# weecology/DeepTreeAttention

Hardware: AMD Instinct MI355X
Metric: patches/sec (train step) Hang2020 369-band 11x11 (higher is better)
Workload: dtype bf16; 1 GPU; Hang2020 spectral+spatial attention train step (fwd + weighted CE + bwd + Adam), bands=369 11x11 classes=200; per_gpu_batch=1024, global_batch=1024, parallelism=dp1, overlap_comm=False, ranks_seen=1

## Files before the change

deeptreeattention_amd/csrc/capi.hip:

```cpp
#include <math.h>
#include <stdlib.h>
#include <stdarg.h>
#include <stdio.h>
#include <string.h>

#include "../../include/dta_hip.h"
#include "kernels.h"
#include "xchg_dev.h"

using namespace dta;

extern "C" {
int dta_xchg_side_args(dta_xchg* x, const double* alpha_g, long long alpha_slot, dta::XchgArgs* out);
void dta_xchg_side_cancel(dta_xchg* x);
}

static thread_local char g_err[512] = "";
void dta_set_error(const char* fmt, ...) {
  va_list ap;
  va_start(ap, fmt);
  vsnprintf(g_err, sizeof(g_err), fmt, ap);
  va_end(ap);
}

// ... 309 lines not shown
  ca.B = p.B; ca.H = p.Hc[L]; ca.W = p.Wc[L]; ca.NC = p.NCin[L]; ca.N = Nconv; ca.Q = p.Qin[L]; ca.HW = p.HWc[L];
  return ca;
}
ConvArgs dgrad_conv_geom(const Plan& p, int L) {
  ConvArgs ca;
  memset(&ca, 0, sizeof(ca));
  ca.B = p.B; ca.H = p.Hc[L]; ca.W = p.Wc[L]; ca.NC = CH[L] / 16; ca.N = CH[L - 1]; ca.Q = p.Qin[L]; ca.HW = p.HWc[L];
  return ca;
}
inline int conv_tab_slot_fwd(int L) { return L; }
inline int conv_tab_slot_dgrad(int L) { return 2 + L; }
void use_conv_tabs(const Plan& p, void* ws, ConvArgs& ca, int G, int slot) {
  if (p.esz != 2) return;
  const int rows = conv_bf16_rows(ca, G);
  if (rows <= 0 || ca.HW > rows) return;
  ca.tabs = reinterpret_cast<const int*>(reinterpret_cast<char*>(ws) + p.rowtabs + (size_t)slot * CONV_TAB_BYTES);
  ca.tabs_rows = rows;
}
bool add_conv_tab_job(const Plan& p, void* ws, const ConvArgs& geom, int G, int slot, ConvTabGroup& tg) {
  ConvArgs ca = geom;
  use_conv_tabs(p, ws, ca, G, slot);
  if (!ca.tabs) return false;
  ConvTabJob& j = tg.job[tg.n++];
  j.HW = ca.HW; j.W = ca.W; j.Q = ca.Q; j.rows = ca.tabs_rows; j.ppw = ca.tabs_rows / ca.HW; j.order = switches().conv_order;
  j.dst = const_cast<int*>(ca.tabs);
  return true;
}

struct LossArgs { const long long* labels; const float* weight; float* loss; float* dlogits; float* scratch; };

struct FwdOpts {
  const void* x_tiles = nullptr;
  const float* gate = nullptr;
  const LossArgs* loss = nullptr;
  bool y0_ready = false;
};
struct BwdOpts {
  int phases = 3;
  const void* x_tiles = nullptr;
  float* dalpha32 = nullptr;
  const float* gate = nullptr;
  dta_xchg* xchg = nullptr;
  long long alpha_slot = -1;
};

bool tail_plan(const Plan& p, const dta_net_desc* d, float* const (*scores)[3]) {
  if (d->kind != DTA_NET_HANG2020 || !d->training || (d->heads_mask & 7) != 4 || (d->heads_mask & DTA_FORWARD_ONLY)) return false;
  if (switches().no_tail || switches().no_lean || !(switches().lean_mask & 1) || switches().bn_inkernel || (switches().fanin & 1)) return false;
  if (scores && (scores[0][2] || scores[1][2])) return false;
  if (p.H != 11 || p.W != 11 || p.F[0][2] != 128 || p.F[1][2] != 512) return false;
  return true;
}

template <typename T>
int forward_t(const Plan& p, const dta_net_desc* d, const dta_subnet_params* nets, const double* alpha,
              const float* const* xs, void* ws, float* const (*scores)[3], float* joint, hipStream_t st,
              const FwdOpts& o) {
  const void* x_tiles = o.x_tiles; const float* gate = o.gate; const LossArgs* loss = o.loss;
  if (o.y0_ready && (d->training || !(d->heads_mask & DTA_FORWARD_ONLY) || p.H != 11 || p.W != 11 || x_tiles)) {
    dta_set_error("a forward on a ready first-conv output needs eval mode, DTA_FORWARD_ONLY and 11x11 patches");
    return 1;
  }
  if (x_tiles && !(p.esz == 2 && p.x_compact && (p.shared_x || p.G == 1))) {
    dta_set_error("input tiles need the bf16 mode, 11x11-class patches and a single input tensor");
    return 1;
  }
  const int G = p.G, B = p.B;
  GemmGroup heads;
  bool tail = tail_plan(p, d, scores);
  if (tail) {
    StageArgs s3 = stage_args(p, d, nets, ws, 2);
    tail = tail_fwd_supported(s3, G, p.classes);
  }
  bool loss_done = false;
  PackWGroup packs;
  SpecPackGroup spacks;
  int pack_mode[3];
  for (int L = 0; L < 3; ++L) {
    const int C = CH[L];
    PackWArgs pw;
    memset(&pw, 0, sizeof(pw));
    const bool cat = L == 0 && p.shared_x;
    pw.G = cat ? 1 : G; pw.NC = p.NCin[L]; pw.N = cat ? 32 * G : C; pw.K = p.Cin[L];
    for (int g = 0; g < G; ++g) pw.src[g] = nets[g].conv_w[L];
    pw.mode = (cat && G == 2) ? 1 : 0; pw.nsplit = 32;
    pack_mode[L] = pw.mode;
    packs.job[packs.n] = pw; packs.dst[packs.n++] = at<char>(ws, p.wp[L]);
    if (L > 0 && d->training) {
      memset(&pw, 0, sizeof(pw));
      pw.G = G; pw.NC = C / 16; pw.N = CH[L - 1]; pw.K = C; pw.mode = 2;
      for (int g = 0; g < G; ++g) pw.src[g] = nets[g].conv_w[L];
      packs.job[packs.n] = pw; packs.dst[packs.n++] = at<char>(ws, p.wd[L]);
    }
    for (int g = 0; g < G; ++g)
      if (p.kinds[g] == KIND_SPECTRAL) {
        int j = spacks.n++;
        spacks.w1[j] = nets[g].att[L][0]; spacks.w2[j] = nets[g].att[L][2];
        spacks.packed[j] = at<float>(ws, p.attpk[g][L]); spacks.C[j] = C; spacks.K[j] = SPEC_K[L];
      }
  }
  const bool reuse = !d->training && (d->heads_mask & DTA_FORWARD_ONLY) && (d->heads_mask & DTA_REUSE_PACKED);
  if (reuse) { packs.n = 0; spacks.n = 0; }
  {
    PrepArgs pa = {};
    pa.nx = (x_tiles || o.y0_ready || fused_input(p)) ? 0 : (p.shared_x ? 1 : G); pa.x_tl_gs = p.x_tl_gs;
    for (int g = 0; g < pa.nx; ++g) pa.x[g] = xs[g];
    pa.x_tl = at<char>(ws, p.x_tl); pa.B = B; pa.C = p.bands; pa.H = p.H; pa.W = p.W;
    pa.x_compact = p.x_compact;
    pa.packs = packs; pa.spacks = spacks;
    if (sizeof(T) == 2 && !reuse) {
      const bool fan_fwd0 = d->training && (switches().fanin & 1);
      for (int L = o.y0_ready ? 1 : 0; L < 3; ++L) add_conv_tab_job(p, ws, fwd_conv_geom(p, d, L, fan_fwd0), (L == 0 && p.shared_x) ? 1 : G, conv_tab_slot_fwd(L), pa.tabs);
      if (d->training && !(d->heads_mask & DTA_FORWARD_ONLY))
        for (int L = 1; L < 3; ++L) add_conv_tab_job(p, ws, dgrad_conv_geom(p, L), G, conv_tab_slot_dgrad(L), pa.tabs);
    }
    if (tail) {
      for (int g = 0; g < 2; ++g) {
        if (!nets[g].fc_w[2] || !nets[g].fc_b[2]) { dta_set_error("Hang2020 forward: the last heads' parameters are missing"); return 1; }
        pa.trans.src[g] = nets[g].fc_w[2];
        pa.trans.dst[g] = at<float>(ws, p.fct) + (size_t)(g ? p.F[0][2] : 0) * p.fct_ld;
        pa.trans.rows[g] = p.classes; pa.trans.cols[g] = p.F[g][2]; pa.trans.ld[g] = p.fct_ld;
      }
      pa.trans.n = 2;
    }
    if (switches().fanin) { pa.zero = at<float>(ws, p.fan_cnt); pa.zero_n4 = (p.fan_cnt_bytes + (d->heads_mask ? p.scores_bytes : 0) + 15) / 16; }
    else { pa.zero = at<float>(ws, p.lead); pa.zero_n4 = (256 + (d->heads_mask ? p.scores_bytes : 0) + 15) / 16; }
    if (launch_forward_prep<T>(pa, st)) return 1;
  }
  for (int L = 0; L < 3; ++L) {
    const int C = CH[L];
    const bool cat = L == 0 && p.shared_x;
    const int Nconv = cat ? 32 * G : C;
    const int launchG = cat ? 1 : G;
    const bool fan_fwd = d->training && (switches().fanin & 1);
    ConvArgs ca = fwd_conv_geom(p, d, L, fan_fwd);
    use_conv_tabs(p, ws, ca, launchG, conv_tab_slot_fwd(L));
    ca.pixel_order = switches().conv_order;
    if (L == 0) {
      ca.x_tl = x_tiles ? x_tiles : at<char>(ws, p.x_tl); ca.x_gs = p.x_tl_gs / p.esz; ca.x_compact = p.x_compact;
      if (!x_tiles && fused_input(p)) {
        for (int g = 0; g < G; ++g) ca.x_nchw[g] = xs[p.shared_x ? 0 : g];
        ca.Cx = p.bands;
        ca.x_tl_out = (d->heads_mask & DTA_FORWARD_ONLY) ? nullptr : at<char>(ws, p.x_tl);
      }
    } else { ca.x_tl = at<char>(ws, p.a_tl[L - 1]); ca.x_gs = (size_t)B * p.NCin[L] * p.Rin[L] * 16; ca.x_compact = p.tl_compact; }
    ca.wp = at<char>(ws, p.wp[L]);
    for (int g = 0; g < G; ++g) ca.bias[g] = nets[g].conv_b[L];
    ca.bias_mode = pack_mode[L]; ca.bias_split = 32;
    ca.y = at<float>(ws, p.y[L]); ca.y_fmt = p.y_fmt;
    if (cat) { ca.y_gs = 0; ca.y_rs = Nconv; } else { ca.y_gs = (size_t)B * p.HWc[L] * C; ca.y_rs = C; }
    ca.stats = d->training ? at<float>(ws, p.stats[L]) : nullptr;
    if (fan_fwd) { ca.fan_count = at<unsigned>(ws, p.fan_ctr) + (size_t)L * MAXG * FAN_R; ca.fan_sums = at<double>(ws, p.fan_fwd[L]); }
    if (!(L == 0 && o.y0_ready)) {
      prof_begin(DTA_SITE_CONV_FWD + L, st);
      if (launch_conv3x3<T>(ca, launchG, st)) return 1;
      prof_end(DTA_SITE_CONV_FWD + L, st);
    }
    BnFinalizeArgs bf;
    memset(&bf, 0, sizeof(bf));
    bf.stats = at<float>(ws, p.stats[L]); bf.nwg = p.nwg[L]; bf.N = Nconv; bf.HW = p.HWc[L]; bf.MWG = p.MWG[L]; bf.B = B;
    for (int g = 0; g < G; ++g) {
      bf.gamma[g] = nets[g].bn_w[L]; bf.beta[g] = nets[g].bn_b[L];
      bf.rmean[g] = nets[g].bn_rm[L]; bf.rvar[g] = nets[g].bn_rv[L]; bf.nbt[g] = nets[g].bn_nbt[L];
    }
    bf.cat_mode = (cat && G == 2); bf.nsplit = 32;
    bf.coef = at<float>(ws, p.coef[L]); bf.training = d->training; bf.momentum = d->bn_momentum; bf.eps = d->bn_eps;
    bf.gate = gate;
    StageArgs sa = stage_args(p, d, nets, ws, L);
    if (fan_fwd) { bf.fsum = ca.fan_sums; sa.bn_inkernel = 1; sa.bnfin = bn_finalize_kargs(bf); }
    else if ((!d->training || switches().bn_inkernel) && p.nwg[L] <= BN_INKERNEL_MAX_NWG) { sa.bn_inkernel = 1; sa.bnfin = bn_finalize_kargs(bf); }
    else if ((switches().lead & 1) && !(L == 2 && tail) && stage_fwd_will_be_lean(sa, G)) {
      sa.bnfin = bn_finalize_kargs(bf);
      sa.lead = G * ((sa.bnfin.C + 7) / 8); sa.lead_flag = at<unsigned>(ws, p.lead) + L; sa.lead_need = (unsigned)sa.lead;
    }
    else if (launch_bn_finalize(bf, G, st)) return 1;
    if (d->heads_mask & DTA_FORWARD_ONLY) sa.attsave = nullptr;
    if (L == 2 && tail) {
      TailArgs ta;
      memset(&ta, 0, sizeof(ta));
      ta.st = sa;
      ta.wt = at<float>(ws, p.fct); ta.ldw = p.fct_ld;
      for (int g = 0; g < 2; ++g) { ta.bias[g] = nets[g].fc_b[2]; ta.scores[g] = at<float>(ws, p.scores[g][2]); }
      ta.alpha = alpha; ta.classes = p.classes;
      ta.ce.gscale = 1.f;
      if (loss) {
        if (!alpha) { dta_set_error("Hang2020 forward + loss needs alpha"); return 1; }
        ta.ce.labels = loss->labels; ta.ce.weight = loss->weight; ta.ce.loss = loss->loss; ta.ce.dlogits = loss->dlogits;
        ta.ce.rowtmp = loss->scratch; ta.ce.joint = joint;
        loss_done = true;
      } else if (!(d->heads_mask & DTA_SKIP_BLEND)) {
        if (!joint || !alpha) { dta_set_error("Hang2020 forward needs head 3, alpha and a joint output"); return 1; }
        ta.ce.joint = joint;
      }
      prof_begin(DTA_SITE_STAGE_FWD + L, st);
      if (launch_tail_fwd(ta, st)) return 1;
      prof_end(DTA_SITE_STAGE_FWD + L, st);
      continue;
    }
    prof_begin(DTA_SITE_STAGE_FWD + L, st);
    if (launch_stage_fwd<T>(sa, G, st)) return 1;
    prof_end(DTA_SITE_STAGE_FWD + L, st);
    if (d->heads_mask & (1 << L)) {
      for (int g = 0; g < G; ++g) {
        if (p.F[g][L] == 0 || nets[g].fc_w[L] == nullptr) continue;
        const int F = p.F[g][L];
        GemmArgs ga;
        memset(&ga, 0, sizeof(ga));
        ga.A = at<float>(ws, p.feat[L]) + (size_t)g * sa.feat_gs; ga.sa_m = F; ga.sa_k = 1;
        ga.Bm = nets[g].fc_w[L]; ga.sb_k = 1; ga.sb_n = F;
        float* out = at<float>(ws, p.scores[g][L]);
        ga.M = B; ga.N = p.cls[g]; ga.K = F; ga.ksplit = min(4, max(1, (F + 63) / 64)); ga.accumulate = 0;
        float* user = (scores && scores[g][L]) ? scores[g][L] : nullptr;
        if (d->kind == DTA_NET_VANILLA && joint) user = joint;
        if (user) {
          out = user;
          if (ga.ksplit > 1) hipMemsetAsync(user, 0, (size_t)B * p.cls[g] * 4, st);
        }
        ga.C = out; ga.sc_m = p.cls[g]; ga.sc_n = 1;
        ga.bias = nets[g].fc_b[L];
        if (!heads.add(ga)) { dta_set_error("too many head GEMMs"); return 1; }
      }
    }
  }
  prof_begin(DTA_SITE_GEMM, st);
  if (launch_gemm_group(heads, st)) return 1;
  prof_end(DTA_SITE_GEMM, st);
  if (tail) return (loss && !loss_done) ? 1 : 0;
  if (loss) {
    BlendCeArgs a;
    memset(&a, 0, sizeof(a));
    a.gscale = 1.f;
    if (d->kind == DTA_NET_HANG2020) {
      if (!alpha || !(d->heads_mask & 4)) { dta_set_error("Hang2020 forward + loss needs head 3 and alpha"); return 1; }
      a.spec = (scores && scores[0][2]) ? scores[0][2] : at<float>(ws, p.scores[0][2]);
      a.spat = (scores && scores[1][2]) ? scores[1][2] : at<float>(ws, p.scores[1][2]);
      a.alpha = alpha; a.joint = joint;
    } else {
      if (!joint) { dta_set_error("forward + loss: the scores of a single-branch network are passed in `joint`"); return 1; }
      a.spec = joint; a.joint = joint;
    }
    a.labels = loss->labels; a.weight = loss->weight; a.dlogits = loss->dlogits; a.loss = loss->loss; a.rowtmp = loss->scratch;
    a.B = B; a.classes = p.classes;
    return launch_blend_ce(a, st);
  }
  if (d->kind == DTA_NET_HANG2020 && !(d->heads_mask & DTA_SKIP_BLEND)) {
    if (!(d->heads_mask & 4) || !joint || !alpha) { dta_set_error("Hang2020 forward needs head 3, alpha and a joint output"); return 1; }
    BlendArgs ba;
    ba.spec = (scores && scores[0][2]) ? scores[0][2] : at<float>(ws, p.scores[0][2]);
    ba.spat = (scores && scores[1][2]) ? scores[1][2] : at<float>(ws, p.scores[1][2]);
    ba.alpha = alpha; ba.joint = joint; ba.B = B; ba.classes = p.classes;
    if (launch_blend(ba, st)) return 1;
  }
  return 0;
}

template <typename T>
int conv_wgrad_layer(const Plan& p, const dta_net_desc* d, const dta_subnet_grads* grads, void* ws, int L,
                     WgradReduceGroup& reduces, hipStream_t st, const BwdOpts& o, const double* dalpha,
                     WgradArgs* defer = nullptr, const WgradArgs* partner = nullptr) {
  const int G = p.G, B = p.B, C = CH[L];
  const bool cat = L == 0 && p.shared_x;
  const int Nconv = cat ? 32 * G : C;
  const int launchG = cat ? 1 : G;
  bool want_w = false;
// ... 1209 lines not shown
```

deeptreeattention_amd/csrc/conv.hip:

```cpp
#include <stdlib.h>

#include "kernels.h"

namespace dta {

template <typename T>
__device__ __forceinline__ void pack_input_block(const float* __restrict__ x, T* __restrict__ out, int B, int C, int H,
                                                 int W, int NC, int CG, int b, int ycg, unsigned char* smem,
                                                 bool compact = false) {
  const int HW = H * W, Q = (H + 2) * (W + 2);
  int* lut = (int*)smem;
  float* sbase = (float*)(lut + ((Q + 3) & ~3));
  const int chunk0 = ycg * CG;
  const int nch = min(CG, NC - chunk0);
  const int c0 = chunk0 * 16;
  const int creal = max(0, min(nch * 16, C - c0));
  const float* src = x + ((size_t)b * C + c0) * HW;
  for (int q = threadIdx.x; q < Q; q += 256) {
    int hh = q / (W + 2) - 1, ww = q % (W + 2) - 1;
    lut[q] = (hh >= 0 && hh < H && ww >= 0 && ww < W) ? hh * W + ww : -1;
  }
  const size_t e0 = ((size_t)b * C + c0) * HW;
  const int phase = (int)(e0 & 3);
  float* s = sbase + phase;
// ... 136 lines not shown
  conv_row_tables<ROWS, 256>(c, rowtab, plq, hist, flag, 0, j.ppw, 0);
  __syncthreads();
  for (int i = threadIdx.x; i < 2 * ROWS; i += 256) j.dst[i] = tab_s[i];
}
__device__ __forceinline__ void conv_tab_job(const ConvTabJob& j) {
  __shared__ int tab_s[2 * 576 + 256 + 4];
  if (j.rows == 256) conv_tab_rows<256>(j, tab_s);
  else if (j.rows == 512) conv_tab_rows<512>(j, tab_s);
  else if (j.rows == 576) conv_tab_rows<576>(j, tab_s);
}

template <typename T>
__global__ __launch_bounds__(256) void k_forward_prep(PrepArgs a) {
  extern __shared__ __attribute__((aligned(16))) unsigned char smem[];
  int y = blockIdx.y;
  if (a.tabs.n > 0) {
    if (y == 0) {
      if ((int)blockIdx.x < a.tabs.n) conv_tab_job(a.tabs.job[blockIdx.x]);
      return;
    }
    y -= 1;
  }
  if (y < a.ncg * a.nx) {
    const int gi = y / a.ncg;
    if ((int)blockIdx.x >= a.B) return;
    pack_input_block<T>(a.x[gi], (T*)((char*)a.x_tl + (size_t)gi * a.x_tl_gs), a.B, a.C, a.H, a.W, a.NC, a.CG, blockIdx.x,
                        y - gi * a.ncg, smem, a.x_compact != 0);
    return;
  }
  y -= a.ncg * a.nx;
  const size_t nthreads = (size_t)gridDim.x * blockDim.x, tid = blockIdx.x * (size_t)blockDim.x + threadIdx.x;
  if (y < a.packs.n) { pack_conv_w_job<T>(a.packs.job[y], (T*)a.packs.dst[y], tid, nthreads); return; }
  y -= a.packs.n;
  if (y < a.spacks.n) { pack_spectral_att_job(a.spacks, y, tid, nthreads); return; }
  y -= a.spacks.n;
  if (y < a.trans.n) { transpose_job(a.trans, y, tid, nthreads); return; }
  y -= a.trans.n;
  if (a.zero) {
    float4* z = (float4*)a.zero;
    for (size_t i = tid; i < a.zero_n4; i += nthreads) z[i] = make_float4(0.f, 0.f, 0.f, 0.f);
  }
}

template <typename T>
int launch_forward_prep(PrepArgs a, hipStream_t st) {
  size_t lds;
  if (pack_input_plan(a.C, a.H, a.W, &a.NC, &a.CG, &lds)) return 1;
  a.ncg = (a.NC + a.CG - 1) / a.CG;
  constexpr int PREP_MIN_BLOCKS = 1024;
  size_t most = a.zero ? a.zero_n4 : 0;
  for (int j = 0; j < a.packs.n; ++j) { const PackWArgs& w = a.packs.job[j]; const size_t e = (size_t)w.G * w.NC * 9 * w.N * 4; if (e > most) most = e; }
  for (int j = 0; j < a.spacks.n; ++j) { const size_t e = (size_t)a.spacks.C[j] * a.spacks.C[j]; if (e > most) most = e; }
  for (int j = 0; j < a.trans.n; ++j) { const size_t e = (size_t)a.trans.cols[j] * a.trans.ld[j]; if (e > most) most = e; }
  int gx = (int)((most + 1023) / 1024);
  gx = gx < 256 ? 256 : (gx > PREP_MIN_BLOCKS ? PREP_MIN_BLOCKS : gx);
  if (a.nx > 0 && gx < a.B) gx = a.B;
  dim3 grid(gx, a.ncg * a.nx + a.packs.n + a.spacks.n + a.trans.n + (a.tabs.n > 0 ? 1 : 0) + (a.zero ? 1 : 0));
  hipLaunchKernelGGL(k_forward_prep<T>, grid, dim3(256), lds, st, a);
  DTA_CHECK_LAUNCH("k_forward_prep");
  return 0;
}
template int launch_forward_prep<float>(PrepArgs, hipStream_t);
template int launch_forward_prep<bf16_t>(PrepArgs, hipStream_t);

template <typename T> struct Frag;
template <> struct Frag<float> {
  static constexpr int KS = 2;
  typedef float reg;
  __device__ static __forceinline__ reg load(const float* rowbase, int row, int ks, int lane) {
    return rowbase[tl_pos<float>(row, ks * 2 + (lane >> 5))];
  }
  __device__ static __forceinline__ f32x16 mfma(reg a, reg b, f32x16 c) {
    return __builtin_amdgcn_mfma_f32_32x32x2f32(a, b, c, 0, 0, 0);
  }
};
template <> struct Frag<bf16_t> {
  static constexpr int KS = 16;
  typedef bf16x8 reg;
  __device__ static __forceinline__ reg load(const bf16_t* rowbase, int row, int ks, int lane) {
    return *reinterpret_cast<const bf16x8*>(rowbase + tl_pos<bf16_t>(row, (lane >> 5) << 3));
  }
  __device__ static __forceinline__ f32x16 mfma(reg a, reg b, f32x16 c) {
    return __builtin_amdgcn_mfma_f32_32x32x16_bf16(a, b, c, 0, 0, 0);
  }
};

template <typename T, int MT, int NT>
__global__ __launch_bounds__(256, 2) void k_conv3x3(ConvArgs a) {
  extern __shared__ __attribute__((aligned(16))) unsigned char smem[];
  constexpr int MWG = 4 * MT * 32;
  constexpr int N = NT * 32;
  int* rowtab = (int*)smem;
  int* plq = rowtab + MWG;
  float* red = (float*)(plq + MWG);
  float* cmean = red + 4 * N;
  T* sx = (T*)(cmean + N);
  const int Q = a.Q, HW = a.HW, W2 = a.W + 2;
  T* sw = sx + (size_t)a.ppw * Q * 16;

  const int tid = threadIdx.x, lane = tid & 63, wave = tid >> 6;
  const int g = blockIdx.y;
  const int pg = blockIdx.x / a.spp, split = blockIdx.x - pg * a.spp;
  const int b0 = pg * a.ppw;
  const int npatch = min(a.ppw, a.B - b0);

  for (int lr = tid; lr < MWG; lr += 256) {
    int pl, pix;
    bool valid;
// ... 389 lines not shown
```

deeptreeattention_amd/csrc/conv_bf16.hip:

```cpp
#include <type_traits>
#include "kernels.h"
#include "xchg_dev.h"

namespace dta {

constexpr int RB = 48;
typedef __attribute__((address_space(3))) s16x4* lds_s16x4_t;

typedef __bf16 hw_bf16x2 __attribute__((ext_vector_type(2)));
__device__ __forceinline__ unsigned cvt_pk_bf16(float lo, float hi) {
  f32x2 v = {lo, hi};
  return __builtin_bit_cast(unsigned, __builtin_convertvector(v, hw_bf16x2));
}

__device__ __forceinline__ int fastdiv(int n, unsigned magic) { return (int)__umulhi((unsigned)n, magic); }
static inline unsigned fastdiv_magic(int d) { return d > 1 ? (unsigned)((0x100000000ull + (unsigned long long)d - 1) / (unsigned long long)d) : 0u; }
__device__ __forceinline__ int fastdiv1(int n, int d, unsigned magic) { return d > 1 ? fastdiv(n, magic) : n; }

__device__ __forceinline__ bf16x8 lds_b128(const unsigned char* base, int off) {
  return *reinterpret_cast<const bf16x8*>(base + off);
}
__device__ __forceinline__ bf16x8 lds_tr8(const unsigned char* base, int off) {
  s16x4 lo = __builtin_amdgcn_ds_read_tr16_b64_v4i16((lds_s16x4_t)(base + off));
  s16x4 hi = __builtin_amdgcn_ds_read_tr16_b64_v4i16((lds_s16x4_t)(base + off + 4 * RB));
// ... 30 lines not shown
#define XS_ACC { xsacc_[0] += xs_[1] - xs_[0]; xsacc_[1] += xs_[2] - xs_[1]; xsacc_[2] += xs_[3] - xs_[2]; }
#define XT(i) xt_[i] = clock64();
#define XT_ACC { _Pragma("unroll") for (int k_ = 0; k_ < 5; ++k_) xacc_[k_] += xt_[k_ + 1] - xt_[k_]; }
#else
#define XT(i)
#define XT_ACC
#define XS(i)
#define XS_ACC
#endif
#ifdef DTA_TICKS
__device__ long long g_cticks[16];
extern "C" int dta_debug_cticks(long long* out) { return (int)hipMemcpyFromSymbol(out, HIP_SYMBOL(g_cticks), sizeof(long long) * 16); }
#define CTICK(i) do { if (!XN && a.N == 64 && a.NC == 2 && a.stats && blockIdx.x == 100 && blockIdx.y == 0 && threadIdx.x == 0) g_cticks[i] = clock64(); } while (0)
#else
#define CTICK(i)
#endif
template <int MT, int NT, bool XN, int NWV = 8, int MINW = 1>
__global__ __launch_bounds__(NWV * 64, MINW) void k_conv3x3_bf16(ConvArgs a) {
  WGSTAMP(XN ? 0 : (a.stats ? (a.N == 64 ? 1 : 2) : -1));
  extern __shared__ __attribute__((aligned(16))) unsigned char smem[];
#ifdef DTA_TICKS
  const long long xentry_ = clock64();
#endif
  CTICK(0);
  constexpr int NW = NWV, NTHR = NW * 64;
  constexpr int MWG = NW * MT * 32;
  constexpr int N = NT * 32;
  constexpr bool TAP_PIPE = true;
  static_assert(!(XN && MT * NT >= 6), "six accumulator tiles + the fp32 staging sets spill (see launch_conv_bf16_t)");
  int* rowtab = (int*)smem;
  int* plq = rowtab + MWG;
  float* red = (float*)(plq + MWG);
  float* cmean = red + NW * N;
  unsigned char* sbuf = (unsigned char*)(cmean + N + NW * N);
  const int Q = a.Q, HW = a.HW, W2 = a.W + 2;
  const int xbytes = a.ppw * Q * RB, wbytes = 9 * N * RB, stage = xbytes + wbytes;
  const bool dbuf = a.dbuf != 0;

  const int tid = threadIdx.x, lane = tid & 63, wave = tid >> 6;
  const int g = blockIdx.y;
  const int pg = a.spp == 1 ? (int)blockIdx.x : (int)blockIdx.x / a.spp, split = blockIdx.x - pg * a.spp;
  const int b0 = pg * a.ppw;
  const int npatch = min(a.ppw, a.B - b0);

  int tab0_[2] = {-1, -1}, tab1_[2] = {0, 0};
  static_assert(MWG <= 2 * NTHR, "two table entries per thread at most");
  if (a.tabs && a.spp == 1 && npatch == a.ppw) {
#pragma unroll
    for (int k = 0; k < 2; ++k)
      if (tid + k * NTHR < MWG) { tab0_[k] = a.tabs[tid + k * NTHR]; tab1_[k] = a.tabs[MWG + tid + k * NTHR]; }
  }
  const int khalf16 = (lane >> 5) * 16;
  int abase[MT];
  const int bbase = (lane & 31) * RB + khalf16;
  const bool xc = a.x_compact != 0;
#define DTA_TABLES \
  { \
    if (a.tabs && a.spp == 1 && npatch == a.ppw) {    \
      _Pragma("unroll") for (int k_ = 0; k_ < 2; ++k_) {                                              \
        const int lr_ = tid + k_ * NTHR;                                                              \
        if (lr_ < MWG) { rowtab[lr_] = tab0_[k_] < 0 ? -1 : b0 * HW + tab0_[k_]; plq[lr_] = tab1_[k_]; } \
      }                                                                                               \
    } else conv_row_tables<MWG, NTHR>(a, rowtab, plq, reinterpret_cast<int*>(red), reinterpret_cast<int*>(cmean), b0, npatch, split); \
    if (xc || XN) {    \
      u32x4* z = reinterpret_cast<u32x4*>(sbuf); \
      const u32x4 zero = {0u, 0u, 0u, 0u}; \
      for (int i = tid; i < xbytes / 16; i += NTHR) { z[i] = zero; if (dbuf) z[i + stage / 16] = zero; } \
    } \
    __syncthreads(); \
_Pragma("unroll") \
    for (int mt = 0; mt < MT; ++mt) { \
      int v = plq[(wave * MT + mt) * 32 + (lane & 31)]; \
      abase[mt] = ((v >> 16) * Q + (v & 0xFFFF)) * RB + khalf16; \
    } \
  }
  if (XN) DTA_TABLES

  f32x16 acc[MT][NT];
#pragma unroll
  for (int mt = 0; mt < MT; ++mt)
#pragma unroll
    for (int nt = 0; nt < NT; ++nt)
#pragma unroll
      for (int r = 0; r < 16; ++r) acc[mt][nt][r] = 0.f;
  float bias[NT];
  if (!XN) {
#pragma unroll
    for (int nt = 0; nt < NT; ++nt) {
      const int n = nt * 32 + (lane & 31);
      float bv = 0.f;
      if (a.bias[0]) {
        if (a.bias_mode == 1) bv = n < a.bias_split ? a.bias[0][n] : a.bias[1][n - a.bias_split];
        else bv = a.bias[g][(a.ncg > 1 ? (int)blockIdx.z : 0) * N + n];
      }
      bias[nt] = bv;
    }
  }

  constexpr int XV = 4, WV = (9 * N * 2 + NTHR - 1) / NTHR;
  const int trows = xc ? HW : Q;
  const int vpp = trows * 2;
  const int nxv = npatch * vpp, wvec = 9 * N * 2;
  const bf16_t* xg = (const bf16_t*)a.x_tl + (size_t)g * a.x_gs + ((size_t)b0 * a.NC) * ((size_t)(a.x_compact ? HW : Q) * 16);
  const int ncg = a.ncg > 1 ? a.ncg : 1, cgi = ncg > 1 ? (int)blockIdx.z : 0, NF = N * ncg;
  const bf16_t* wg = (const bf16_t*)a.wp + (size_t)g * a.NC * 9 * NF * 16;
  const size_t xchunk = (size_t)trows * 16;
  unsigned xsrc[XV];
  int xdst[XV], wdst[WV];
#pragma unroll
  for (int u = 0; u < XV; ++u) {
    int v = min(tid + u * NTHR, max(nxv, 1) - 1);
    int pl = fastdiv(v, a.m_vpp), o = v - pl * vpp;
    int row = o >> 1;
    if (xc) { const int hh = fastdiv(row, a.m_W); row = (hh + 1) * W2 + (row - hh * a.W) + 1; }
    xsrc[u] = (unsigned)(((size_t)pl * a.NC) * xchunk + (size_t)o * 8);
    xdst[u] = (pl * Q + row) * RB + (o & 1) * 16;
  }
  constexpr int QV = 2 * MT;
  constexpr bool xn = XN;
  const float* xf = xn ? a.x_nchw[g] + (size_t)b0 * a.Cx * HW : nullptr;
  const int nquad = xn ? npatch * 4 * HW : 0;
  unsigned qsrc[QV];
  int qdst[QV], qch[QV];
#pragma unroll
  for (int u = 0; u < QV; ++u) {
    int q = min(tid + u * NTHR, max(nquad, 1) - 1);
// ... 34 lines not shown
    _Pragma("unroll") for (int u = 0; u < WV; ++u) rw[u] = swp_[wsrc(u)];                             \
  }
#define DTA_STORE(sx_, sw_, chunk_)                                                                   \
  {                                                                                                   \
    if (xn) {                                                                                         \
      _Pragma("unroll") for (int u = 0; u < QV; ++u) {                                                \
         \
                        \
        u32x2 pk_;                                                                                    \
        pk_.x = cvt_pk_bf16(rf[u][0], rf[u][1]);                                                      \
        pk_.y = cvt_pk_bf16(rf[u][2], rf[u][3]);                                                      \
        if (tid + u * NTHR < nquad) *reinterpret_cast<u32x2*>((sx_) + qdst[u]) = pk_;                 \
      }                                                                                               \
    } else {                                                                                          \
      _Pragma("unroll") for (int u = 0; u < XV; ++u)                                                  \
          if (tid + u * NTHR < nxv) *reinterpret_cast<u32x4*>((sx_) + xdst[u]) = rx[u];               \
    }                                                                                                 \
    _Pragma("unroll") for (int u = 0; u < WV; ++u)                                                    \
        if (tid + u * NTHR < wvec) *reinterpret_cast<u32x4*>((sw_) + wdst[u]) = rw[u];                \
  }
#define DTA_TAP_LOAD(set_, tap_, sx_, sw_)                                                            \
  {                                                                                                   \
    const int toffB_ = (((tap_) / 3) * W2 + ((tap_) % 3)) * RB;                                       \
    _Pragma("unroll") for (int mt = 0; mt < MT; ++mt) af[set_][mt] = lds_b128((sx_), abase[mt] + toffB_); \
    _Pragma("unroll") for (int nt = 0; nt < NT; ++nt)                                                 \
        bf[set_][nt] = lds_b128((sw_), bbase + ((tap_) * N + nt * 32) * RB);                          \
  }
#define DTA_COMPUTE(sx_, sw_)                                                                         \
  if constexpr (TAP_PIPE) {                                                                           \
    bf16x8 af[2][MT], bf[2][NT];                                                                      \
    DTA_TAP_LOAD(0, 0, sx_, sw_)                                                                      \
    DTA_TAP_LOAD(1, 1, sx_, sw_)                                                                      \
    _Pragma("unroll") for (int tap = 0; tap < 9; ++tap) {                                             \
      _Pragma("unroll") for (int mt = 0; mt < MT; ++mt)                                               \
        _Pragma("unroll") for (int nt = 0; nt < NT; ++nt)                                             \
            acc[mt][nt] = __builtin_amdgcn_mfma_f32_32x32x16_bf16(af[tap & 1][mt], bf[tap & 1][nt], acc[mt][nt], 0, 0, 0); \
      if (tap + 2 < 9) DTA_TAP_LOAD(tap & 1, tap + 2, sx_, sw_)                                       \
    }                                                                                                 \
    __builtin_amdgcn_sched_group_barrier(0x100, 2 * (MT + NT), 0);                                    \
    _Pragma("unroll") for (int tap = 0; tap < 9; ++tap) {                                             \
      __builtin_amdgcn_sched_group_barrier(0x008, MT * NT, 0);                                        \
      if (tap + 2 < 9) __builtin_amdgcn_sched_group_barrier(0x100, MT + NT, 0);                       \
    }                                                                                                 \
  } else {                                                                                            \
    _Pragma("unroll") for (int tap = 0; tap < 9; ++tap) {                                             \
      bf16x8 af[1][MT], bf[1][NT];                                                                    \
      DTA_TAP_LOAD(0, tap, sx_, sw_)                                                                  \
      _Pragma("unroll") for (int mt = 0; mt < MT; ++mt)                                               \
        _Pragma("unroll") for (int nt = 0; nt < NT; ++nt)                                             \
            acc[mt][nt] = __builtin_amdgcn_mfma_f32_32x32x16_bf16(af[0][mt], bf[0][nt], acc[mt][nt], 0, 0, 0); \
    }                                                                                                 \
  }

  if (XN && dbuf) {
    float rg[QV][4];
#define DTA_FETCH_XF(dst_, chunk_)                                                                    \
    _Pragma("unroll") for (int u = 0; u < QV; ++u)                                                    \
      _Pragma("unroll") for (int j = 0; j < 4; ++j) {                                                 \
        const int ch_ = min(min((chunk_), a.NC - 1) * 16 + qch[u] + j, a.Cx - 1);                     \
        dst_[u][j] = __builtin_nontemporal_load(xf + qsrc[u] + (size_t)ch_ * HW);    \
      }
#define DTA_STORE_XF(src_, sx_)                                                                       \
    _Pragma("unroll") for (int u = 0; u < QV; ++u) {                                                  \
      u32x2 pk_;                                                                                      \
      pk_.x = cvt_pk_bf16(src_[u][0], src_[u][1]);                                                    \
      pk_.y = cvt_pk_bf16(src_[u][2], src_[u][3]);                                                    \
      if (tid + u * NTHR < nquad) *reinterpret_cast<u32x2*>((sx_) + qdst[u]) = pk_;                   \
    }
#define DTA_FETCH_W(chunk_)                                                                           \
    {                                                                                                 \
      const u32x4* swp_ = reinterpret_cast<const u32x4*>(wg + (size_t)min((chunk_), a.NC - 1) * 9 * NF * 16); \
      _Pragma("unroll") for (int u = 0; u < WV; ++u) rw[u] = swp_[wsrc(u)];                           \
    }
#define DTA_STORE_W(sw_)                                                                              \
    _Pragma("unroll") for (int u = 0; u < WV; ++u)                                                    \
        if (tid + u * NTHR < wvec) *reinterpret_cast<u32x4*>((sw_) + wdst[u]) = rw[u];
#define DTA_TILE_OUT(cx_, chunk_)                                                                     \
    if (xo) {    \
                 \
      _Pragma("unroll") for (int u = 0; u < XV; ++u)                                                  \
        if (tid + u * NTHR < nxv)                                                                     \
          *reinterpret_cast<u32x4*>(xo + xsrc[u] + (size_t)(chunk_) * xchunk) = *reinterpret_cast<const u32x4*>((cx_) + xdst[u]); \
    }
    DTA_FETCH_XF(rf, 0)
    DTA_FETCH_W(0)
    DTA_STORE_XF(rf, sbuf)
    DTA_STORE_W(sbuf + xbytes)
    if (a.NC > 1) {
      DTA_FETCH_XF(rf, 1)
      DTA_FETCH_W(1)
    }
    if (a.NC > 2) DTA_FETCH_XF(rg, 2)
    __syncthreads();
    unsigned char* s0 = sbuf;
    unsigned char* s1 = sbuf + stage;
    const bool late = !(a.pixel_order & 2) && __builtin_amdgcn_readfirstlane(wave) >= NW / 2;
#ifdef DTA_TICKS
    long long xt_[6] = {0, 0, 0, 0, 0, 0}, xacc_[5] = {0, 0, 0, 0, 0}, xs_[4] = {0, 0, 0, 0}, xsacc_[3] = {0, 0, 0};
    const long long xt0_ = clock64();
    if (blockIdx.x == 100 && blockIdx.y == 0 && tid == 0) g_xticks[0][6] = xt0_ - xentry_;
#endif
    for (int chunk = 0; chunk < a.NC; chunk += 2) {
      XT(0)
      DTA_TILE_OUT(s0, chunk)
      XT(1)
      if (late) { DTA_COMPUTE(s0, s0 + xbytes) }
      XT(2)
      if (chunk + 1 < a.NC) {
        XS(0)
        DTA_STORE_XF(rf, s1)
        XS(1)
        DTA_STORE_W(s1 + xbytes)
        XS(2)
        if (chunk + 2 < a.NC) DTA_FETCH_W(chunk + 2)
        if (chunk + 3 < a.NC) DTA_FETCH_XF(rf, chunk + 3)
        XS(3)
        XS_ACC
      }
      XT(3)
      if (!late) { DTA_COMPUTE(s0, s0 + xbytes) }
      XT(4)
      __syncthreads();
      XT(5)
      XT_ACC
      if (chunk + 1 >= a.NC) break;
      XT(0)
      DTA_TILE_OUT(s1, chunk + 1)
      XT(1)
      if (late) { DTA_COMPUTE(s1, s1 + xbytes) }
      XT(2)
      if (chunk + 2 < a.NC) {
        XS(0)
        DTA_STORE_XF(rg, s0)
        XS(1)
        DTA_STORE_W(s0 + xbytes)
        XS(2)
        if (chunk + 3 < a.NC) DTA_FETCH_W(chunk + 3)
        if (chunk + 4 < a.NC) DTA_FETCH_XF(rg, chunk + 4)
        XS(3)
        XS_ACC
      }
      XT(3)
      if (!late) { DTA_COMPUTE(s1, s1 + xbytes) }
      XT(4)
      __syncthreads();
      XT(5)
      XT_ACC
    }
#ifdef DTA_TICKS
    if (blockIdx.x == 100 && blockIdx.y == 0 && lane == 0 && (wave == 0 || wave == NW / 2)) {
      long long* o_ = g_xticks[wave ? 1 : 0];
      for (int k_ = 0; k_ < 5; ++k_) o_[k_] = xacc_[k_];
      o_[5] = clock64() - xt0_;
      for (int k_ = 0; k_ < 3; ++k_) g_xticks2[wave ? 1 : 0][k_] = xsacc_[k_];
    }
#endif
#undef DTA_TILE_OUT
#undef DTA_STORE_W
#undef DTA_FETCH_W
#undef DTA_STORE_XF
#undef DTA_FETCH_XF
  } else {
  DTA_FETCH(0)
  if (!XN) DTA_TABLES
  DTA_STORE(sbuf, sbuf + xbytes, 0)
  if (a.NC > 1) DTA_FETCH(1)
  __syncthreads();
  CTICK(2);
  const bool late2 = dbuf && !(a.pixel_order & 2) && __builtin_amdgcn_readfirstlane(wave) >= NW / 2;
  for (int chunk = 0; chunk < a.NC; ++chunk) {
    unsigned char* cx = sbuf + ((dbuf && (chunk & 1)) ? stage : 0);
    unsigned char* nx = sbuf + ((dbuf && !(chunk & 1)) ? stage : 0);
    const bool more = chunk + 1 < a.NC;
    if (xo) {
#pragma unroll
      for (int u = 0; u < XV; ++u)
        if (tid + u * NTHR < nxv)
          *reinterpret_cast<u32x4*>(xo + xsrc[u] + (size_t)chunk * xchunk) = *reinterpret_cast<const u32x4*>(cx + xdst[u]);
    }
    if (late2) { DTA_COMPUTE(cx, cx + xbytes) }
    if (dbuf && more) {
      DTA_STORE(nx, nx + xbytes, chunk + 1)
      if (chunk + 2 < a.NC) DTA_FETCH(chunk + 2)
    }
    if (!late2) { DTA_COMPUTE(cx, cx + xbytes) }
    __syncthreads();
    if (!dbuf && more) {
      DTA_STORE(nx, nx + xbytes, chunk + 1)
      if (chunk + 2 < a.NC) DTA_FETCH(chunk + 2)
      __syncthreads();
    }
  }
  }
#undef DTA_COMPUTE
#undef DTA_TAP_LOAD
#undef DTA_TABLES
#undef DTA_STORE
#undef DTA_FETCH

  CTICK(3);
#ifdef DTA_TICKS
  const long long xloopend_ = clock64();
#endif
  if (XN) {
#pragma unroll
    for (int nt = 0; nt < NT; ++nt) {
      int n = nt * 32 + (lane & 31);
      float bv = 0.f;
      if (a.bias[0]) {
        if (a.bias_mode == 1) bv = n < a.bias_split ? a.bias[0][n] : a.bias[1][n - a.bias_split];
        else bv = a.bias[g][cgi * N + n];
      }
      bias[nt] = bv;
    }
  }
  float s1[NT], s2[NT], shiftK[NT];
#pragma unroll
  for (int nt = 0; nt < NT; ++nt) { s1[nt] = 0.f; s2[nt] = 0.f; shiftK[nt] = 0.f; }
  float* red2 = cmean + N;
  if (a.stats) {
    if (wave == 0 && lane < 32) {
      const bool v0 = rowtab[0] >= 0;
#pragma unroll
      for (int nt = 0; nt < NT; ++nt) cmean[nt * 32 + lane] = bias[nt] + (v0 ? acc[0][nt][0] : 0.f);
    }
    __syncthreads();
#pragma unroll
    for (int nt = 0; nt < NT; ++nt) shiftK[nt] = cmean[nt * 32 + (lane & 31)];
  }
  float* yg = a.y + (size_t)g * a.y_gs + cgi * N;
  if (a.y_fmt == FMT_F32) {
#pragma unroll
    for (int mt = 0; mt < MT; ++mt) {
#pragma unroll
      for (int r = 0; r < 16; ++r) {
        int lr = (wave * MT + mt) * 32 + (r & 3) + 8 * (r >> 2) + 4 * (lane >> 5);
        int orow = rowtab[lr];
#pragma unroll
        for (int nt = 0; nt < NT; ++nt) {
          float v = acc[mt][nt][r] + bias[nt];
          if (orow >= 0) {
            yg[(size_t)orow * a.y_rs + nt * 32 + (lane & 31)] = v;
            const float d = v - shiftK[nt];
            s1[nt] += d; s2[nt] += d * d;
          }
        }
      }
    }
  } else {
    unsigned short* y16 = reinterpret_cast<unsigned short*>(a.y) + (size_t)g * a.y_gs + cgi * N;
    const bool odd = lane & 1;
    const int ncol = (lane & 31) & ~1;
    constexpr int EP = N * 2 + 16;
    unsigned char* E = sbuf;
    auto pack_tile = [&](auto fmt_tag) {
    constexpr int YFMT = decltype(fmt_tag)::value;
#pragma unroll
    for (int mt = 0; mt < MT; ++mt) {
#pragma unroll
      for (int r = 0; r < 16; r += 2) {
        const int lr0 = (wave * MT + mt) * 32 + (r & 3) + 8 * (r >> 2) + 4 * (lane >> 5);
        const int orow0 = rowtab[lr0], orow1 = rowtab[lr0 + 1];
#pragma unroll
        for (int nt = 0; nt < NT; ++nt) {
          const float v0 = acc[mt][nt][r] + bias[nt], v1 = acc[mt][nt][r + 1] + bias[nt];
          const float d0 = v0 - shiftK[nt], d1 = v1 - shiftK[nt];
          if (orow0 >= 0) { s1[nt] += d0; s2[nt] += d0 * d0; }
          if (orow1 >= 0) { s1[nt] += d1; s2[nt] += d1 * d1; }
          const float got = lane_xor1(odd ? v0 : v1);
          const unsigned pk = odd ? pack2_fmt(got, v1, YFMT) : pack2_fmt(v0, got, YFMT);
          *reinterpret_cast<unsigned*>(E + (lr0 + (odd ? 1 : 0)) * EP + (nt * 32 + ncol) * 2) = pk;
        }
      }
    }
    };
    CTICK(6);
    if (a.y_fmt == FMT_F16) pack_tile(std::integral_constant<int, FMT_F16>{});
    else pack_tile(std::integral_constant<int, FMT_BF16>{});
    CTICK(7);
    __syncthreads();
    CTICK(8);
    constexpr int VPR = N / 8;
#pragma unroll
    for (int u = 0; u < MWG * VPR / NTHR; ++u) {
      const int v = tid + u * NTHR, row = v / VPR, part = v % VPR;
      const int orow = rowtab[row];
      if (orow >= 0)
        *reinterpret_cast<u32x4*>(y16 + (size_t)orow * a.y_rs + part * 8) = *reinterpret_cast<const u32x4*>(E + row * EP + part * 16);
    }
  }
  CTICK(4);
#ifdef DTA_TICKS
  if (XN && blockIdx.x == 100 && blockIdx.y == 0 && tid == 0) g_xticks[0][7] = clock64() - xloopend_;
#endif
  if (a.stats == nullptr) return;
  const int cnt = (a.spp == 1) ? npatch * HW : min(MWG, HW - split * MWG);
#pragma unroll
  for (int nt = 0; nt < NT; ++nt) {
    const float u1 = s1[nt] + __shfl_xor(s1[nt], 32), u2 = s2[nt] + __shfl_xor(s2[nt], 32);
    if (lane < 32) { red[wave * N + nt * 32 + lane] = u1; red2[wave * N + nt * 32 + lane] = u2; }
  }
  __syncthreads();
  if (tid < N) {
    float t1 = 0.f, t2 = 0.f;
#pragma unroll
    for (int w = 0; w < NW; ++w) { t1 += red[w * N + tid]; t2 += red2[w * N + tid]; }
    const float dm = t1 / (float)cnt;
    const float mean = cmean[tid] + dm;
    float m2 = t2 - t1 * dm;
    m2 = m2 > 0.f ? m2 : 0.f;
    cmean[tid] = mean;
    float* o = a.stats + (((size_t)g * gridDim.x + blockIdx.x) * NF + cgi * N + tid) * 2;
    if (a.fan_count) fan_store2(o, cmean[tid], m2);
    else { o[0] = cmean[tid]; o[1] = m2; }
  }
  CTICK(5);
#ifdef DTA_TICKS
  if (XN && blockIdx.x == 100 && blockIdx.y == 0 && tid == 0) g_xticks[1][7] = clock64() - xloopend_;
#endif
  if (a.fan_count) conv_stats_fanin<NTHR>(a, g, N, HW, MWG, reinterpret_cast<double*>(sbuf), reinterpret_cast<int*>(cmean));
}

template <int MT, int NT, int NW = 8, int MINW = 1>
static int launch_conv_bf16_t(ConvArgs a, int G, hipStream_t st) {
  constexpr int MWG = NW * MT * 32, N = NT * 32;
  int nwg;
  conv_geometry(a.HW, MWG, a.B, &a.ppw, &a.spp, &nwg);
  if (a.tabs_rows != MWG) a.tabs = nullptr;
  a.m_vpp = fastdiv_magic((a.x_compact ? a.HW : a.Q) * 2); a.m_W = fastdiv_magic(a.W); a.m_HW = fastdiv_magic(a.HW); a.m_4HW = fastdiv_magic(4 * a.HW);
  size_t tab = (size_t)MWG * 8 + (size_t)17 * N * 4, stage = ((size_t)a.ppw * a.Q + (size_t)9 * N) * RB;
  a.dbuf = tab + 2 * stage <= 160 * 1024 && a.NC > 4;
  size_t lds = tab + (a.dbuf ? 2 : 1) * stage;
  if (a.y_fmt != FMT_F32) {
    const size_t epi = tab + (size_t)MWG * (N * 2 + 16);
    if (epi > lds) lds = epi;
  }
  if (lds > 160 * 1024) { dta_set_error("conv3x3(bf16): LDS need %zu B exceeds 160 KiB (H=%d W=%d)", lds, a.H, a.W); return 1; }
  if ((a.ppw < a.B ? a.ppw : a.B) * a.Q * 2 > 4 * NW * 64) { dta_set_error("conv3x3(bf16): %dx%d tile exceeds the staging plan", a.H, a.W); return 1; }
  static DevOnce attr_once;
  if (attr_once.first()) {
    hipFuncSetAttribute((const void*)k_conv3x3_bf16<MT, NT, false, NW, MINW>, hipFuncAttributeMaxDynamicSharedMemorySize, 160 * 1024);
    if constexpr (MT * NT < 6) hipFuncSetAttribute((const void*)k_conv3x3_bf16<MT, NT, true, NW>, hipFuncAttributeMaxDynamicSharedMemorySize, 160 * 1024);
  }
  if (a.x_nchw[0]) {
    if (a.spp != 1) { dta_set_error("conv3x3(bf16): the fused-input first conv needs whole patches per workgroup"); return 1; }
    if constexpr (MT * NT < 6) hipLaunchKernelGGL((k_conv3x3_bf16<MT, NT, true, NW>), dim3(nwg, G), dim3(NW * 64), lds, st, a);
    else { dta_set_error("conv3x3(bf16): no fused-input kernel for %d-row x %d-column workgroups", MWG, N); return 1; }
  } else {
    hipLaunchKernelGGL((k_conv3x3_bf16<MT, NT, false, NW, MINW>), dim3(nwg, G, a.ncg > 1 ? a.ncg : 1), dim3(NW * 64), lds, st, a);
  }
  DTA_CHECK_LAUNCH("k_conv3x3_bf16");
  return 0;
}

int conv_mwg_bf16(int N, int HW) {
  if (N == 32 && HW > 512) {
    const int r512 = (HW + 511) / 512 * 512, r576 = (HW + 575) / 576 * 576;
    if (r576 < r512) return 576;
  }
  return conv_mwg(N);
}

int conv_bf16_rows(const ConvArgs& a, int G) {
  switch (a.N) {
    case 32: return (a.mwg == 576 || (a.stats == nullptr && conv_mwg_bf16(32, a.HW) == 576)) ? 576 : 512;
    case 64: {
      int ppw, spp, nwg;
      conv_geometry(a.HW, 512, a.B, &ppw, &spp, &nwg);
      if (a.stats == nullptr && nwg * G <= 128) return 256;
      return a.mwg == 256 ? 256 : a.mwg == 576 ? 576 : 512;
    }
    case 128: return (a.ncg == 2 && a.mwg == 576) ? 576 : 256;
// ... 480 lines not shown
```

Measured before the change: 1.960 million patches/s.

## Trim conv epilogue syncs, narrow prep zeroing, skip unused feature writes

The bf16 conv epilogue now builds per-row validity bitmasks with ballots and publishes the BN shift inside the last mainloop barrier. This removes a separate __syncthreads and the rowtab reads from the epilogue, and the stats reduction is folded into the existing pack-tile barrier. Forward prep now zeroes only the score buffers that k-split head GEMMs accumulate into, and uses a larger minimum grid. Stages that need no head features get a null feat pointer so those stores are skipped. Several unrelated changes are bundled, and the shared LDS reuse (vbits in red, kfull in plq) adds aliasing risk.

After: 1.962 million patches/s (median of 5 runs). Within noise of the previous version (+0.1%).

```diff
diff --git a/deeptreeattention_amd/csrc/capi.hip b/deeptreeattention_amd/csrc/capi.hip
--- a/deeptreeattention_amd/csrc/capi.hip
+++ b/deeptreeattention_amd/csrc/capi.hip
@@ -385,6 +385,8 @@
   return true;
 }
 
+static inline int head_ksplit(int F) { return min(4, max(1, (F + 63) / 64)); }
+
 template <typename T>
 int forward_t(const Plan& p, const dta_net_desc* d, const dta_subnet_params* nets, const double* alpha,
               const float* const* xs, void* ws, float* const (*scores)[3], float* joint, hipStream_t st,
@@ -456,8 +458,18 @@
       }
       pa.trans.n = 2;
     }
-    if (switches().fanin) { pa.zero = at<float>(ws, p.fan_cnt); pa.zero_n4 = (p.fan_cnt_bytes + (d->heads_mask ? p.scores_bytes : 0) + 15) / 16; }
-    else { pa.zero = at<float>(ws, p.lead); pa.zero_n4 = (256 + (d->heads_mask ? p.scores_bytes : 0) + 15) / 16; }
+    size_t zscores = 0;
+    for (int L = 0; L < 3; ++L) {
+      if (!(d->heads_mask & (1 << L)) || (L == 2 && tail)) continue;
+      for (int g = 0; g < G; ++g) {
+        if (p.F[g][L] == 0 || nets[g].fc_w[L] == nullptr || head_ksplit(p.F[g][L]) <= 1) continue;
+        if ((scores && scores[g][L]) || (d->kind == DTA_NET_VANILLA && joint)) continue;
+        const size_t end = p.scores[g][L] + (size_t)B * p.cls[g] * 4 - p.scores_all;
+        if (end > zscores) zscores = end;
+      }
+    }
+    if (switches().fanin) { pa.zero = at<float>(ws, p.fan_cnt); pa.zero_n4 = (p.fan_cnt_bytes + zscores + 15) / 16; }
+    else { pa.zero = at<float>(ws, p.lead); pa.zero_n4 = (256 + zscores + 15) / 16; }
     if (launch_forward_prep<T>(pa, st)) return 1;
   }
   for (int L = 0; L < 3; ++L) {
@@ -500,6 +512,11 @@
     bf.coef = at<float>(ws, p.coef[L]); bf.training = d->training; bf.momentum = d->bn_momentum; bf.eps = d->bn_eps;
     bf.gate = gate;
     StageArgs sa = stage_args(p, d, nets, ws, L);
+    {
+      bool want_feat = (d->heads_mask & (1 << L)) != 0;
+      for (int g = 0; g < G; ++g) want_feat |= scores && scores[g][L];
+      if (!want_feat) sa.feat = nullptr;
+    }
     if (fan_fwd) { bf.fsum = ca.fan_sums; sa.bn_inkernel = 1; sa.bnfin = bn_finalize_kargs(bf); }
     else if ((!d->training || switches().bn_inkernel) && p.nwg[L] <= BN_INKERNEL_MAX_NWG) { sa.bn_inkernel = 1; sa.bnfin = bn_finalize_kargs(bf); }
     else if ((switches().lead & 1) && !(L == 2 && tail) && stage_fwd_will_be_lean(sa, G)) {
@@ -542,7 +559,7 @@
         ga.A = at<float>(ws, p.feat[L]) + (size_t)g * sa.feat_gs; ga.sa_m = F; ga.sa_k = 1;
         ga.Bm = nets[g].fc_w[L]; ga.sb_k = 1; ga.sb_n = F;
         float* out = at<float>(ws, p.scores[g][L]);
-        ga.M = B; ga.N = p.cls[g]; ga.K = F; ga.ksplit = min(4, max(1, (F + 63) / 64)); ga.accumulate = 0;
+        ga.M = B; ga.N = p.cls[g]; ga.K = F; ga.ksplit = head_ksplit(F); ga.accumulate = 0;
         float* user = (scores && scores[g][L]) ? scores[g][L] : nullptr;
         if (d->kind == DTA_NET_VANILLA && joint) user = joint;
         if (user) {
diff --git a/deeptreeattention_amd/csrc/conv.hip b/deeptreeattention_amd/csrc/conv.hip
--- a/deeptreeattention_amd/csrc/conv.hip
+++ b/deeptreeattention_amd/csrc/conv.hip
@@ -212,8 +212,9 @@
   for (int j = 0; j < a.packs.n; ++j) { const PackWArgs& w = a.packs.job[j]; const size_t e = (size_t)w.G * w.NC * 9 * w.N * 4; if (e > most) most = e; }
   for (int j = 0; j < a.spacks.n; ++j) { const size_t e = (size_t)a.spacks.C[j] * a.spacks.C[j]; if (e > most) most = e; }
   for (int j = 0; j < a.trans.n; ++j) { const size_t e = (size_t)a.trans.cols[j] * a.trans.ld[j]; if (e > most) most = e; }
+  constexpr int PREP_FLOOR_BLOCKS = 320;
   int gx = (int)((most + 1023) / 1024);
-  gx = gx < 256 ? 256 : (gx > PREP_MIN_BLOCKS ? PREP_MIN_BLOCKS : gx);
+  gx = gx < PREP_FLOOR_BLOCKS ? PREP_FLOOR_BLOCKS : (gx > PREP_MIN_BLOCKS ? PREP_MIN_BLOCKS : gx);
   if (a.nx > 0 && gx < a.B) gx = a.B;
   dim3 grid(gx, a.ncg * a.nx + a.packs.n + a.spacks.n + a.trans.n + (a.tabs.n > 0 ? 1 : 0) + (a.zero ? 1 : 0));
   hipLaunchKernelGGL(k_forward_prep<T>, grid, dim3(256), lds, st, a);
diff --git a/deeptreeattention_amd/csrc/conv_bf16.hip b/deeptreeattention_amd/csrc/conv_bf16.hip
--- a/deeptreeattention_amd/csrc/conv_bf16.hip
+++ b/deeptreeattention_amd/csrc/conv_bf16.hip
@@ -106,6 +106,8 @@
   }
   const int khalf16 = (lane >> 5) * 16;
   int abase[MT];
+  unsigned vmask[MT];
+  unsigned long long* vbits = reinterpret_cast<unsigned long long*>(red);
   const int bbase = (lane & 31) * RB + khalf16;
   const bool xc = a.x_compact != 0;
 #define DTA_TABLES \
@@ -114,8 +116,18 @@
       _Pragma("unroll") for (int k_ = 0; k_ < 2; ++k_) {                                              \
         const int lr_ = tid + k_ * NTHR;                                                              \
         if (lr_ < MWG) { rowtab[lr_] = tab0_[k_] < 0 ? -1 : b0 * HW + tab0_[k_]; plq[lr_] = tab1_[k_]; } \
+        const unsigned long long vb_ = __ballot(tab0_[k_] >= 0);       \
+        if (lane == 0 && lr_ < MWG) vbits[lr_ >> 6] = vb_;                                            \
       }                                                                                               \
-    } else conv_row_tables<MWG, NTHR>(a, rowtab, plq, reinterpret_cast<int*>(red), reinterpret_cast<int*>(cmean), b0, npatch, split); \
+    } else {                                                                                          \
+      conv_row_tables<MWG, NTHR>(a, rowtab, plq, reinterpret_cast<int*>(red), reinterpret_cast<int*>(cmean), b0, npatch, split); \
+      __syncthreads();                                                                                \
+      _Pragma("unroll") for (int k_ = 0; k_ < 2; ++k_) {                                              \
+        const int lr_ = tid + k_ * NTHR;                                                              \
+        const unsigned long long vb_ = __ballot(lr_ < MWG && rowtab[lr_ < MWG ? lr_ : 0] >= 0);       \
+        if (lane == 0 && lr_ < MWG) vbits[lr_ >> 6] = vb_;                                            \
+      }                                                                                               \
+    }                                                                                                 \
     if (xc || XN) {    \
       u32x4* z = reinterpret_cast<u32x4*>(sbuf); \
       const u32x4 zero = {0u, 0u, 0u, 0u}; \
@@ -126,6 +138,10 @@
     for (int mt = 0; mt < MT; ++mt) { \
       int v = plq[(wave * MT + mt) * 32 + (lane & 31)]; \
       abase[mt] = ((v >> 16) * Q + (v & 0xFFFF)) * RB + khalf16; \
+       \
+       \
+       \
+      vmask[mt] = __builtin_amdgcn_readfirstlane(reinterpret_cast<const unsigned*>(vbits)[wave * MT + mt]); \
     } \
   }
   if (XN) DTA_TABLES
@@ -266,6 +282,11 @@
     }                                                                                                 \
   }
 
+#define DTA_PUT_SHIFT                                                                                 \
+  if (a.stats && wave == 0 && lane < 32) {                                                            \
+    _Pragma("unroll") for (int nt = 0; nt < NT; ++nt) cmean[nt * 32 + lane] = (vmask[0] & 1u) ? acc[0][nt][0] : 0.f; \
+  }
+
   if (XN && dbuf) {
     float rg[QV][4];
 #define DTA_FETCH_XF(dst_, chunk_)                                                                    \
@@ -334,6 +355,7 @@
       XT(3)
       if (!late) { DTA_COMPUTE(s0, s0 + xbytes) }
       XT(4)
+      if (chunk + 1 >= a.NC) DTA_PUT_SHIFT
       __syncthreads();
       XT(5)
       XT_ACC
@@ -357,6 +379,7 @@
       XT(3)
       if (!late) { DTA_COMPUTE(s1, s1 + xbytes) }
       XT(4)
+      if (chunk + 2 >= a.NC) DTA_PUT_SHIFT
       __syncthreads();
       XT(5)
       XT_ACC
@@ -398,6 +421,7 @@
       if (chunk + 2 < a.NC) DTA_FETCH(chunk + 2)
     }
     if (!late2) { DTA_COMPUTE(cx, cx + xbytes) }
+    if (!more) DTA_PUT_SHIFT
     __syncthreads();
     if (!dbuf && more) {
       DTA_STORE(nx, nx + xbytes, chunk + 1)
@@ -406,6 +430,7 @@
     }
   }
   }
+#undef DTA_PUT_SHIFT
 #undef DTA_COMPUTE
 #undef DTA_TAP_LOAD
 #undef DTA_TABLES
@@ -432,16 +457,39 @@
 #pragma unroll
   for (int nt = 0; nt < NT; ++nt) { s1[nt] = 0.f; s2[nt] = 0.f; shiftK[nt] = 0.f; }
   float* red2 = cmean + N;
+  float* kfull = reinterpret_cast<float*>(plq);
   if (a.stats) {
+#pragma unroll
+    for (int nt = 0; nt < NT; ++nt) shiftK[nt] = bias[nt] + cmean[nt * 32 + (lane & 31)];
     if (wave == 0 && lane < 32) {
-      const bool v0 = rowtab[0] >= 0;
-#pragma unroll
-      for (int nt = 0; nt < NT; ++nt) cmean[nt * 32 + lane] = bias[nt] + (v0 ? acc[0][nt][0] : 0.f);
-    }
-    __syncthreads();
-#pragma unroll
-    for (int nt = 0; nt < NT; ++nt) shiftK[nt] = cmean[nt * 32 + (lane & 31)];
-  }
+#pragma unroll
+      for (int nt = 0; nt < NT; ++nt) kfull[nt * 32 + lane] = shiftK[nt];
+    }
+  }
+  auto put_partials = [&]() __attribute__((always_inline)) {
+#pragma unroll
+    for (int nt = 0; nt < NT; ++nt) {
+      const float u1 = s1[nt] + __shfl_xor(s1[nt], 32), u2 = s2[nt] + __shfl_xor(s2[nt], 32);
+      if (lane < 32) { red[wave * N + nt * 32 + lane] = u1; red2[wave * N + nt * 32 + lane] = u2; }
+    }
+  };
+  auto fold_partials = [&]() __attribute__((always_inline)) {
+    const int cnt = (a.spp == 1) ? npatch * HW : min(MWG, HW - split * MWG);
+    float t1 = 0.f, t2 = 0.f;
+#pragma unroll
+    for (int w = 0; w < NW; ++w) { t1 += red[w * N + tid]; t2 += red2[w * N + tid]; }
+    const float dm = t1 / (float)cnt;
+    const float mean = kfull[tid] + dm;
+    float m2 = t2 - t1 * dm;
+    m2 = m2 > 0.f ? m2 : 0.f;
+    cmean[tid] = mean;
+    float* o = a.stats + (((size_t)g * gridDim.x + blockIdx.x) * NF + cgi * N + tid) * 2;
+    if (a.fan_count) fan_store2(o, mean, m2);
+    else { o[0] = mean; o[1] = m2; }
+  };
+  unsigned vrow[MT];
+#pragma unroll
+  for (int mt = 0; mt < MT; ++mt) vrow[mt] = vmask[mt] >> (4 * (lane >> 5));
   float* yg = a.y + (size_t)g * a.y_gs + cgi * N;
   if (a.y_fmt == FMT_F32) {
 #pragma unroll
@@ -450,16 +498,23 @@
       for (int r = 0; r < 16; ++r) {
         int lr = (wave * MT + mt) * 32 + (r & 3) + 8 * (r >> 2) + 4 * (lane >> 5);
         int orow = rowtab[lr];
+        const bool ok = (vrow[mt] >> ((r & 3) + 8 * (r >> 2))) & 1u;
 #pragma unroll
         for (int nt = 0; nt < NT; ++nt) {
           float v = acc[mt][nt][r] + bias[nt];
-          if (orow >= 0) {
+          if (ok) {
             yg[(size_t)orow * a.y_rs + nt * 32 + (lane & 31)] = v;
             const float d = v - shiftK[nt];
             s1[nt] += d; s2[nt] += d * d;
           }
         }
       }
+    }
+    CTICK(4);
+    if (a.stats) {
+      put_partials();
+      __syncthreads();
+      if (tid < N) fold_partials();
     }
   } else {
     unsigned short* y16 = reinterpret_cast<unsigned short*>(a.y) + (size_t)g * a.y_gs + cgi * N;
@@ -474,15 +529,16 @@
 #pragma unroll
       for (int r = 0; r < 16; r += 2) {
         const int lr0 = (wave * MT + mt) * 32 + (r & 3) + 8 * (r >> 2) + 4 * (lane >> 5);
-        const int orow0 = rowtab[lr0], orow1 = rowtab[lr0 + 1];
+        const bool ok0 = (vrow[mt] >> ((r & 3) + 8 * (r >> 2))) & 1u, ok1 = (vrow[mt] >> ((r & 3) + 8 * (r >> 2) + 1)) & 1u;
 #pragma unroll
         for (int nt = 0; nt < NT; ++nt) {
           const float v0 = acc[mt][nt][r] + bias[nt], v1 = acc[mt][nt][r + 1] + bias[nt];
           const float d0 = v0 - shiftK[nt], d1 = v1 - shiftK[nt];
-          if (orow0 >= 0) { s1[nt] += d0; s2[nt] += d0 * d0; }
-          if (orow1 >= 0) { s1[nt] += d1; s2[nt] += d1 * d1; }
+          if (ok0) { s1[nt] += d0; s2[nt] += d0 * d0; }
+          if (ok1) { s1[nt] += d1; s2[nt] += d1 * d1; }
           const float got = lane_xor1(odd ? v0 : v1);
-          const unsigned pk = odd ? pack2_fmt(got, v1, YFMT) : pack2_fmt(v0, got, YFMT);
+          const float lo = odd ? got : v0, hi = odd ? v1 : got;
+          const unsigned pk = pack2_fmt(lo, hi, YFMT);
           *reinterpret_cast<unsigned*>(E + (lr0 + (odd ? 1 : 0)) * EP + (nt * 32 + ncol) * 2) = pk;
         }
       }
@@ -491,9 +547,15 @@
     CTICK(6);
     if (a.y_fmt == FMT_F16) pack_tile(std::integral_constant<int, FMT_F16>{});
     else pack_tile(std::integral_constant<int, FMT_BF16>{});
+    if (a.stats) put_partials();
     CTICK(7);
     __syncthreads();
     CTICK(8);
+    if (a.stats && tid < N) fold_partials();
+    CTICK(5);
+#ifdef DTA_TICKS
+    if (XN && blockIdx.x == 100 && blockIdx.y == 0 && tid == 0) g_xticks[1][7] = clock64() - xloopend_;
+#endif
     constexpr int VPR = N / 8;
 #pragma unroll
     for (int u = 0; u < MWG * VPR / NTHR; ++u) {
@@ -502,36 +564,12 @@
       if (orow >= 0)
         *reinterpret_cast<u32x4*>(y16 + (size_t)orow * a.y_rs + part * 8) = *reinterpret_cast<const u32x4*>(E + row * EP + part * 16);
     }
-  }
-  CTICK(4);
+    CTICK(4);
+  }
 #ifdef DTA_TICKS
   if (XN && blockIdx.x == 100 && blockIdx.y == 0 && tid == 0) g_xticks[0][7] = clock64() - xloopend_;
 #endif
   if (a.stats == nullptr) return;
-  const int cnt = (a.spp == 1) ? npatch * HW : min(MWG, HW - split * MWG);
-#pragma unroll
-  for (int nt = 0; nt < NT; ++nt) {
-    const float u1 = s1[nt] + __shfl_xor(s1[nt], 32), u2 = s2[nt] + __shfl_xor(s2[nt], 32);
-    if (lane < 32) { red[wave * N + nt * 32 + lane] = u1; red2[wave * N + nt * 32 + lane] = u2; }
-  }
-  __syncthreads();
-  if (tid < N) {
-    float t1 = 0.f, t2 = 0.f;
-#pragma unroll
-    for (int w = 0; w < NW; ++w) { t1 += red[w * N + tid]; t2 += red2[w * N + tid]; }
-    const float dm = t1 / (float)cnt;
-    const float mean = cmean[tid] + dm;
-    float m2 = t2 - t1 * dm;
-    m2 = m2 > 0.f ? m2 : 0.f;
-    cmean[tid] = mean;
-    float* o = a.stats + (((size_t)g * gridDim.x + blockIdx.x) * NF + cgi * N + tid) * 2;
-    if (a.fan_count) fan_store2(o, cmean[tid], m2);
-    else { o[0] = cmean[tid]; o[1] = m2; }
-  }
-  CTICK(5);
-#ifdef DTA_TICKS
-  if (XN && blockIdx.x == 100 && blockIdx.y == 0 && tid == 0) g_xticks[1][7] = clock64() - xloopend_;
-#endif
   if (a.fan_count) conv_stats_fanin<NTHR>(a, g, N, HW, MWG, reinterpret_cast<double*>(sbuf), reinterpret_cast<int*>(cmean));
 }
 
```
